# itshawi/data-accelerator

Hardware: AMD Instinct MI355X
Metric: events/sec (node) + p99 latency, SimulatedData IoT Flow (higher is better)
Workload: dtype fp64/int64 columns (no reduced precision)

## Files before the change

### dxa/io/kafka_device.py

```python
from __future__ import annotations

import ctypes
from dataclasses import dataclass
from typing import List, Optional, Sequence, Tuple

import numpy as np
import torch

_PLAN_ERRS = {-2: "message format is not v2", -3: "CRC mismatch", -5: "codec decoded on the host only",
              -7: "malformed compressed payload (LZ4 / snappy / zstd)", -8: "dependent-block LZ4 frame", -9: "offset deltas with gaps"}


TORCH_DT = {np.dtype(np.int32): torch.int32, np.dtype(np.int64): torch.int64, np.dtype(np.uint8): torch.uint8}


class Unsupported(Exception):
    """The fetch needs the host decoder."""


_BOUND = False


def _lib():
    global _BOUND
# ... 213 lines not shown
    keep[cut] = max_records - before
    keep[cut + 1:] = 0
    q = FetchPlan(**{**p.__dict__, "b_keep": keep.astype(np.int32)})
    q.b_rec0 = _rec0(q)
    q.next_offset = int(p.b_base[cut] + p.b_skip[cut] + keep[cut])
    return q


class DeviceRecordDecoder:

    def __init__(self, device, chunks: int = 4, copy_stream=None, decode_stream=None, track: bool = True,
                 verify_crc: bool = False):
        self.device = torch.device(device)
        self.verify_crc = verify_crc
        self.crc_stream = torch.cuda.Stream(self.device) if verify_crc else None
        self.chunks = max(1, chunks)
        cus = torch.cuda.get_device_properties(self.device).multi_processor_count
        self.min_blocks_per_chunk = cus * 64
        self.copy_stream = copy_stream or torch.cuda.Stream(self.device)
        self.decode_stream = decode_stream or torch.cuda.Stream(self.device)
        self.track = track
        self.checks: List["DecodeStatus"] = []

    def decode(self, staging: torch.Tensor, plan: FetchPlan):
        from ..engine.processor import RawBatch
        from ..ops import native as N
        dev = self.device
        n = plan.nrec
        if plan.packed is None:
            if not hasattr(self, "_packs"):
                self._packs = PlanBufferPool()
            pb = self._packs.get()
            plan.buffer = pb
            arrs, layout, used = pb.carve(plan.nbat, plan.nblk)
            for name, _dt, _k in _ARRAYS:
                arrs[name][...] = getattr(plan, name)
            packed = pb.buf[:used]
        else:
            packed, layout = plan.packed, plan.layout
        with torch.cuda.stream(self.copy_stream):
            dtab = packed.to(dev, non_blocking=True)
            ddata = torch.empty(plan.nbytes + 32, dtype=torch.uint8, device=dev)
            tab_ev = torch.cuda.Event()
            tab_ev.record(self.copy_stream)
        if getattr(plan, "buffer", None) is not None:
            plan.buffer.release(tab_ev)
        views = {name: dtab[off:off + cnt * np.dtype(dt).itemsize].view(TORCH_DT[np.dtype(dt)])
                 for (name, off, cnt), (_, dt, _k) in zip(layout, _ARRAYS)}
        tabs = [views[k] for k in ("k_comp_off", "k_comp_len", "k_stored", "k_out_off", "k_cap", "b_count",
                                   "b_skip", "b_keep", "b_first", "b_nblk", "b_rec0")]
        crc_tabs = [views[k] for k in ("b_crc_off", "b_crc_len", "b_crc")]
        co, cl, sd, oo, cap, bc, bs, bk, bf, bn, br = tabs
        with torch.cuda.stream(self.decode_stream):
            out = torch.empty(plan.out_bytes + 64, dtype=torch.uint8, device=dev)
            produced = torch.empty(max(1, plan.nblk), dtype=torch.int64, device=dev)
            bstat = torch.empty(max(1, plan.nblk), dtype=torch.int32, device=dev)
            offs = torch.empty(n + 1, dtype=torch.int64, device=dev)
            ends = torch.empty(max(1, n), dtype=torch.int64, device=dev)
            rstat = torch.empty(max(1, plan.nbat), dtype=torch.int32, device=dev)
        self.decode_stream.wait_event(tab_ev)
        st = self.decode_stream.cuda_stream
        nb = plan.nblk
        chunks = max(1, min(self.chunks, nb // max(1, self.min_blocks_per_chunk)))
        kinds = set(np.unique(plan.k_stored[:nb]).tolist()) if nb else set()
        has_gzip, has_snappy, has_zstd = 2 in kinds, 3 in kinds, 4 in kinds
        bounds = np.linspace(0, nb, chunks + 1).astype(np.int64)
        ev_last = tab_ev
        copied = 0
        for k in range(chunks):
            b0, b1 = int(bounds[k]), int(bounds[k + 1])
            if b1 <= b0:
                continue
            lo = copied
            hi = plan.nbytes if b1 == nb else int(plan.k_comp_off[b1])
            copied = hi
            N.call("dxa_memcpy_h2d_async", ddata.data_ptr() + lo, staging.data_ptr() + lo, hi - lo,
                   self.copy_stream.cuda_stream)
            ev = torch.cuda.Event()
            ev.record(self.copy_stream)
            ev_last = ev
            self.decode_stream.wait_event(ev)
            N.call("dxa_lz4_decode_into", N.ptr(ddata), N.ptr(co[b0:b1]), N.ptr(cl[b0:b1]), N.ptr(sd[b0:b1]),
                   N.ptr(oo[b0:b1]), N.ptr(cap[b0:b1]), b1 - b0, N.ptr(out), N.ptr(produced[b0:b1]),
                   N.ptr(bstat[b0:b1]), st)
            for present, entry in ((has_gzip, "dxa_inflate_into"), (has_snappy, "dxa_snappy_decode_into"),
                                   (has_zstd, "dxa_zstd_decode_into")):
                if present:
                    N.call(entry, N.ptr(ddata), N.ptr(co[b0:b1]), N.ptr(cl[b0:b1]), N.ptr(sd[b0:b1]),
                           N.ptr(oo[b0:b1]), N.ptr(cap[b0:b1]), b1 - b0, N.ptr(out), N.ptr(produced[b0:b1]),
                           N.ptr(bstat[b0:b1]), st)
        with torch.cuda.stream(self.decode_stream):
            offs[n:].fill_(plan.out_bytes)
        N.call("dxa_kafka_records", N.ptr(out), plan.nbat, N.ptr(bc), N.ptr(bs), N.ptr(bk), N.ptr(bf), N.ptr(bn),
               N.ptr(br), N.ptr(oo), N.ptr(cap), N.ptr(produced), N.ptr(bstat), N.ptr(offs), N.ptr(ends),
               N.ptr(rstat), st)
        done = torch.cuda.Event()
        done.record(self.decode_stream)
        if self.verify_crc:
            cs = self.crc_stream
            cs.wait_event(ev_last)
            with torch.cuda.stream(cs):
                cstat = torch.empty(max(1, plan.nbat), dtype=torch.int32, device=dev)
            N.call("dxa_kafka_crc", N.ptr(ddata), plan.nbat, *[N.ptr(t) for t in crc_tabs], N.ptr(cstat),
                   cs.cuda_stream)
            cs.wait_event(done)
            with torch.cuda.stream(cs):
                bad = (rstat[:plan.nbat] != 0).sum() + (cstat[:plan.nbat] != 0).sum()
                status = DecodeStatus(bad, cs)
            for t in (ddata, dtab, rstat):
                t.record_stream(cs)
        else:
            with torch.cuda.stream(self.decode_stream):
                status = DecodeStatus((rstat[:plan.nbat] != 0).sum(), self.decode_stream)
        for t in (ddata, produced, bstat, dtab):
            t.record_stream(self.decode_stream)
        if self.track:
            self.checks.append(status)
        self._inflight = [(e, b) for e, b in getattr(self, "_inflight", []) if not e.query()] + \
            [(status.event if self.verify_crc else done, (staging, packed))]
        return RawBatch(out, offs, n, ends=ends[:n], source_bytes=plan.nbytes, status=status), done

    def check(self):
        pending, self.checks = self.checks, []
        bad = sum(s.failed() for s in pending)
        if bad:
            raise DecodeError(f"{bad} Kafka record batch(es) failed to decode on the device")


class DecodeError(ValueError):
    pass


class DecodeStatus:

    __slots__ = ("host", "event")

    def __init__(self, bad: torch.Tensor, stream):
        self.host = torch.empty(1, dtype=torch.int64, pin_memory=True)
        self.host.copy_(bad.reshape(1), non_blocking=True)
        self.event = torch.cuda.Event()
        self.event.record(stream)

    def failed(self) -> int:
        self.event.synchronize()
        return int(self.host[0])

    def raise_if_failed(self, what: str = "batch"):
        bad = self.failed()
        if bad:
            raise DecodeError(f"{what}: {bad} Kafka record batch(es) failed to decode on the device")


_CRC_POLY = 0x82F63B78


def _multmodp(a: int, b: int) -> int:
    p = 0
    m = 1 << 31
    while m:
        if a & m:
            p ^= b
        b = (b >> 1) ^ _CRC_POLY if b & 1 else b >> 1
        m >>= 1
    return p


def _x2n_table():
# ... 116 lines not shown
```

### dxa/ops/csrc/lz4.hip

```cpp
#include "dxa_common.h"

namespace {

struct InWin {
  const uint8_t* base;
  uintptr_t wb;
  uint4 w;
  __device__ __forceinline__ uint32_t at(int64_t q) {
    const uintptr_t a = reinterpret_cast<uintptr_t>(base + q);
    const uintptr_t b = a & ~(uintptr_t)15;
    if (b != wb) {
      wb = b;
      w = *reinterpret_cast<const uint4*>(b);
    }
    return dxa::window_byte(w, (uint32_t)(a - b));
  }
};

struct OutBuf {
  uint8_t* p;
  int64_t len;
  int head;
  int nacc;
  uint64_t a0, a1;
// ... 27 lines not shown
      const int k = (int)(q - acc0);
      return (uint32_t)(((k < 8) ? (a0 >> (8 * k)) : (a1 >> (8 * (k - 8)))) & 0xff);
    }
    const uintptr_t a = reinterpret_cast<uintptr_t>(p + q);
    const uintptr_t b = a & ~(uintptr_t)15;
    if (b != wb) {
      wb = b;
      asm volatile("" ::: "memory");
      w = *reinterpret_cast<const uint4*>(b);
    }
    return dxa::window_byte(w, (uint32_t)(a - b));
  }
  __device__ __forceinline__ void finish() {
    uint8_t* q = p + len - nacc;
    for (int k = 0; k < nacc; ++k) q[k] = (uint8_t)((k < 8 ? a0 >> (8 * k) : a1 >> (8 * (k - 8))) & 0xff);
  }
};

enum : int32_t { LZ_OK = 0, LZ_TRUNC = 1, LZ_OFFSET = 2, LZ_OVERFLOW = 3, LZ_SIZE = 4 };

template <bool WRITE>
__device__ int32_t run_block(const uint8_t* src, int64_t n, uint8_t* dst, int64_t cap, int64_t& produced) {
  InWin in{src, 0, make_uint4(0, 0, 0, 0)};
  OutBuf out;
  if (WRITE) out.init(dst);
  int64_t ip = 0, op = 0;
  while (ip < n) {
    const uint32_t token = in.at(ip++);
    int64_t lit = token >> 4;
    if (lit == 15) {
      uint32_t b;
      do { if (ip >= n) return LZ_TRUNC; b = in.at(ip++); lit += b; } while (b == 255);
    }
    if (lit > n - ip) return LZ_TRUNC;
    if (lit > cap - op) return LZ_OVERFLOW;
    if (WRITE) for (int64_t k = 0; k < lit; ++k) out.put(in.at(ip + k));
    ip += lit;
    op += lit;
    if (ip >= n) break;
    if (n - ip < 2) return LZ_TRUNC;
    const int64_t off = (int64_t)in.at(ip) | ((int64_t)in.at(ip + 1) << 8);
    ip += 2;
    if (off == 0 || off > op) return LZ_OFFSET;
    int64_t ml = token & 15;
    if (ml == 15) {
      uint32_t b;
      do { if (ip >= n) return LZ_TRUNC; b = in.at(ip++); ml += b; } while (b == 255);
    }
    ml += 4;
    if (ml > cap - op) return LZ_OVERFLOW;
    if (WRITE) {
      const int64_t s = op - off;
      if (off == 1) {
        const uint32_t c = out.get(s);
        for (int64_t k = 0; k < ml; ++k) out.put(c);
      } else {
        for (int64_t k = 0; k < ml; ++k) out.put(out.get(s + k));
      }
    }
    op += ml;
  }
  if (WRITE) out.finish();
  produced = op;
  return LZ_OK;
}

__global__ __launch_bounds__(256) void lz4_sizes_kernel(const uint8_t* __restrict__ src,
                                                        const int64_t* __restrict__ comp_off,
                                                        const int32_t* __restrict__ comp_len,
                                                        const uint8_t* __restrict__ stored, int64_t nb,
                                                        int64_t max_block, int64_t* __restrict__ out_len,
                                                        int32_t* __restrict__ status) {
  const int64_t b = (int64_t)blockIdx.x * blockDim.x + threadIdx.x;
  if (b >= nb) return;
  if (stored[b]) { out_len[b] = comp_len[b]; status[b] = LZ_OK; return; }
  int64_t produced = 0;
  const int32_t rc = run_block<false>(src + comp_off[b], comp_len[b], nullptr, max_block, produced);
  out_len[b] = rc == LZ_OK ? produced : 0;
  status[b] = rc;
}

constexpr int kWaitVm0 = 0xF70;

template <int G>
__global__ __launch_bounds__(256) void lz4_decode_group_kernel(const uint8_t* __restrict__ src,
                                                               const int64_t* __restrict__ comp_off,
                                                               const int32_t* __restrict__ comp_len,
                                                               const uint8_t* __restrict__ stored,
                                                               const int64_t* __restrict__ out_off,
                                                               const int64_t* __restrict__ out_len, int64_t nb,
                                                               uint8_t* __restrict__ dst,
                                                               int32_t* __restrict__ status,
                                                               int64_t* __restrict__ produced) {
  static_assert(G == 8 || G == 16, "group width");
  constexpr int NW = 16 / G, LPL = 16 / G, BPL = 32 / G, LOG_G = G == 8 ? 3 : 4;
  constexpr int WB = 64, PIPE = 32;
  const int64_t b = ((int64_t)blockIdx.x * 256 + threadIdx.x) / G;
  const int gl = (int)(threadIdx.x & (G - 1));
  const int gbase = (int)((threadIdx.x & 63) & ~(G - 1));
  if (b >= nb) return;
  const uint8_t kd = stored[b];
  if (kd > 1) return;
  const int32_t n = comp_len[b];
  const int64_t cap64 = out_len[b];
  const uint8_t* in = src + comp_off[b];
  uint8_t* out = dst + out_off[b];
  auto put = [&](bool on, int32_t pos, uint32_t v) {
    if (on) out[pos] = (uint8_t)v;
  };
  auto fetch = [&](bool on, int32_t pos) -> uint32_t { return on ? (uint32_t)out[pos] : 0u; };
  if (kd) {
    if (produced ? (n > cap64) : (n != cap64)) {
      if (gl == 0) status[b] = LZ_SIZE;
      return;
    }
    for (int32_t k = gl; k < n; k += G) out[k] = in[k];
    if (gl == 0) {
      status[b] = LZ_OK;
      if (produced) produced[b] = n;
    }
    return;
  }
  if (cap64 > INT32_MAX || cap64 < 0 || n < 0) {
    if (gl == 0) status[b] = LZ_OVERFLOW;
    return;
  }
  const int32_t cap = (int32_t)cap64;
  const int32_t shift = (int32_t)(reinterpret_cast<uintptr_t>(in) & 3);
  const uint8_t* a0 = in - shift;
  const int32_t lim = shift + n + 16;
  uint32_t X[NW];
  auto ld = [&](int32_t w0) {
#pragma unroll
    for (int k = 0; k < NW; ++k) {
      const int32_t q = w0 + 4 * (gl + G * k);
      X[k] = (q + 4 <= lim) ? *reinterpret_cast<const uint32_t*>(a0 + q) : 0u;
    }
    __builtin_amdgcn_s_waitcnt(kWaitVm0);
  };
  auto wbyte = [&](int32_t r) -> uint32_t {
    const int d = (r >> 2) & (G * NW - 1);
    const int addr = (gbase + (d & (G - 1))) << 2;
    uint32_t v = (uint32_t)__builtin_amdgcn_ds_bpermute(addr, (int)X[0]);
    if constexpr (NW == 2) {
      const uint32_t v1 = (uint32_t)__builtin_amdgcn_ds_bpermute(addr, (int)X[1]);
      v = (d >> LOG_G) ? v1 : v;
    }
    return (v >> ((r & 3) * 8)) & 0xffu;
  };
  int32_t xb = 0;
  ld(0);
  auto get = [&](int32_t p) -> uint32_t {
    if (p - xb >= WB) {
      xb = p & ~3;
      ld(xb);
    }
    return wbyte(p - xb);
  };
  const int32_t iend = shift + n;
  int32_t ip = shift, op = 0, rc = LZ_OK, done = 0;
  int32_t pdst = 0, pml = 0;
  uint32_t pv[BPL];
#pragma unroll
  for (int k = 0; k < BPL; ++k) pv[k] = 0;
  auto flush = [&]() {
#pragma unroll
    for (int k = 0; k < BPL; ++k) put(gl + G * k < pml, pdst + G * k + gl, pv[k]);
  };
  while (ip < iend) {
    if (ip - xb > WB - 16) {
      xb = ip & ~3;
      ld(xb);
    }
    const int32_t r = ip - xb;
    const uint32_t token = wbyte(r);
    int32_t lit = (int32_t)(token >> 4);
    const int32_t mlc = (int32_t)(token & 15);
    const bool has_ext = mlc == 15 && lit < 15 && r + lit + 4 <= WB;
    const uint32_t mext = has_ext ? wbyte(r + lit + 3) : 0u;
    const int32_t fml = mlc + 4 + (int32_t)mext;
    const int32_t fhdr = lit + 3 + (mlc == 15 ? 1 : 0);
    if (lit < 15 && (mlc < 15 || mext < 255) && r + fhdr <= WB && iend - ip >= fhdr && cap - op >= lit + fml) {
#pragma unroll
      for (int k = 0; k < LPL; ++k) {
        const uint32_t lv = wbyte(r + 1 + G * k + gl);
        put(gl + G * k < lit, op + G * k + gl, lv);
      }
      const int32_t off = (int32_t)(wbyte(r + 1 + lit) | (wbyte(r + 2 + lit) << 8));
      ip += fhdr;
      op += lit;
      if (off == 0 || off > op) { rc = LZ_OFFSET; break; }
      const int32_t ml = fml;
      const int32_t s0 = op - off;
      const int32_t src_end = s0 + (off < ml ? off : ml);
      if (pml > 0 && (src_end > pdst || ml > PIPE)) {
        flush();
        pml = 0;
      }
      if (src_end > done) {
        __builtin_amdgcn_s_waitcnt(kWaitVm0);
        asm volatile("" ::: "memory");
        done = pml > 0 ? pdst : op;
      }
      if (ml > PIPE) {
        if (off >= ml) {
          for (int32_t c = 0; c < ml; c += G)
            if (c + gl < ml) out[op + c + gl] = out[s0 + c + gl];
        } else {
          for (int32_t c = 0; c < ml; c += G) {
            const uint32_t i = (uint32_t)(c + gl);
            if ((int32_t)i < ml) out[op + i] = out[s0 + (int32_t)(i % (uint32_t)off)];
          }
        }
        op += ml;
        continue;
      }
      uint32_t v[BPL];
      if (off >= ml) {
#pragma unroll
        for (int k = 0; k < BPL; ++k) v[k] = fetch(gl + G * k < ml, s0 + G * k + gl);
      } else {
        const uint32_t o = (uint32_t)off;
#pragma unroll
        for (int k = 0; k < BPL; ++k) v[k] = fetch(gl + G * k < ml, s0 + (int32_t)((uint32_t)(gl + G * k) % o));
      }
      if (pml > 0) flush();
      pdst = op;
      pml = ml;
#pragma unroll
      for (int k = 0; k < BPL; ++k) pv[k] = v[k];
      op += ml;
      continue;
    }
    if (pml > 0) {
      flush();
      pml = 0;
    }
    ++ip;
    if (lit == 15) {
      uint32_t e;
      do {
        if (ip >= iend) { rc = LZ_TRUNC; break; }
        e = get(ip);
        ++ip;
        lit += (int32_t)e;
      } while (e == 255);
      if (rc != LZ_OK) break;
    }
    if (lit > iend - ip) { rc = LZ_TRUNC; break; }
    if (lit > cap - op) { rc = LZ_OVERFLOW; break; }
    for (int32_t c = 0; c < lit; c += G)
      if (c + gl < lit) out[op + c + gl] = a0[ip + c + gl];
    ip += lit;
    op += lit;
    if (ip >= iend) break;
    if (iend - ip < 2) { rc = LZ_TRUNC; break; }
    const int32_t off = (int32_t)(get(ip) | (get(ip + 1) << 8));
    ip += 2;
    if (off == 0 || off > op) { rc = LZ_OFFSET; break; }
    int32_t ml = mlc;
    if (ml == 15) {
      uint32_t e;
      do {
        if (ip >= iend) { rc = LZ_TRUNC; break; }
        e = get(ip);
        ++ip;
        ml += (int32_t)e;
      } while (e == 255);
      if (rc != LZ_OK) break;
    }
    ml += 4;
    if (ml > cap - op) { rc = LZ_OVERFLOW; break; }
    const int32_t s0 = op - off;
    if (s0 + (off < ml ? off : ml) > done) {
      __builtin_amdgcn_s_waitcnt(kWaitVm0);
      asm volatile("" ::: "memory");
      done = op;
    }
    if (off >= ml) {
      for (int32_t c = 0; c < ml; c += G)
        if (c + gl < ml) out[op + c + gl] = out[s0 + c + gl];
    } else {
      for (int32_t c = 0; c < ml; c += G) {
        const uint32_t i = (uint32_t)(c + gl);
        if ((int32_t)i < ml) out[op + i] = out[s0 + (int32_t)(i % (uint32_t)off)];
      }
    }
    op += ml;
  }
  if (pml > 0) flush();
  if (rc == LZ_OK && !produced && op != cap) rc = LZ_SIZE;
  if (gl == 0) {
    status[b] = rc;
    if (produced) produced[b] = op;
  }
}

}

DXA_API int dxa_lz4_block_sizes(const void* src, const void* comp_off, const void* comp_len, const void* stored,
                                int64_t nb, int64_t max_block, void* out_len, void* status, void* st) {
  if (nb <= 0) return 0;
  hipLaunchKernelGGL(lz4_sizes_kernel, dim3((unsigned)((nb + 255) / 256)), dim3(256), 0, (hipStream_t)st,
                     (const uint8_t*)src, (const int64_t*)comp_off, (const int32_t*)comp_len, (const uint8_t*)stored,
                     nb, max_block, (int64_t*)out_len, (int32_t*)status);
  return (int)hipGetLastError();
}

template <int G>
static int launch_group(int64_t nb, hipStream_t s, const uint8_t* src, const int64_t* co, const int32_t* cl,
                        const uint8_t* sd, const int64_t* oo, const int64_t* ol, uint8_t* dst, int32_t* status,
                        int64_t* produced) {
  const dim3 grid((unsigned)((nb * G + 255) / 256));
  hipLaunchKernelGGL((lz4_decode_group_kernel<G>), grid, dim3(256), 0, s, src, co, cl, sd, oo, ol, nb, dst, status,
                     produced);
  return (int)hipGetLastError();
}

DXA_API int dxa_lz4_decode(const void* src, const void* comp_off, const void* comp_len, const void* stored,
                           const void* out_off, const void* out_len, int64_t nb, int64_t max_out, void* dst,
                           void* status, void* st) {
  if (nb <= 0) return 0;
  const hipStream_t s = (hipStream_t)st;
  return launch_group<16>(nb, s, (const uint8_t*)src, (const int64_t*)comp_off, (const int32_t*)comp_len,
                          (const uint8_t*)stored, (const int64_t*)out_off, (const int64_t*)out_len, (uint8_t*)dst,
                          (int32_t*)status, (int64_t*)nullptr);
}

DXA_API int dxa_lz4_decode_into(const void* src, const void* comp_off, const void* comp_len, const void* stored,
                                const void* out_off, const void* cap, int64_t nb, void* dst, void* produced,
                                void* status, void* st) {
  if (nb <= 0) return 0;
  const hipStream_t s = (hipStream_t)st;
  const uint8_t* s8 = (const uint8_t*)src;
  const int64_t* co = (const int64_t*)comp_off;
  const int32_t* cl = (const int32_t*)comp_len;
  const uint8_t* sd = (const uint8_t*)stored;
  const int64_t* oo = (const int64_t*)out_off;
  const int64_t* cp = (const int64_t*)cap;
  return launch_group<16>(nb, s, s8, co, cl, sd, oo, cp, (uint8_t*)dst, (int32_t*)status, (int64_t*)produced);
}

DXA_API int dxa_memcpy_h2d_async(void* dst, const void* src, int64_t n, void* st) {
  if (n <= 0) return 0;
  return (int)hipMemcpyAsync(dst, src, (size_t)n, hipMemcpyHostToDevice, (hipStream_t)st);
}
```

### dxa/ops/lz4.py

```python
from __future__ import annotations

import ctypes
import os
from dataclasses import dataclass
from typing import Optional

import numpy as np
import torch

from . import native as N

DEFAULT_BLOCK = 16 * 1024
_HOST = None


class Lz4Error(RuntimeError):
    pass


def _host():
    global _HOST
    if _HOST is None:
        from .serialize import lib
        L = lib()
# ... 102 lines not shown
            return None
        return off, ln


def frame_table(data) -> FrameTable:
    a = _as_np(data)
    L = _host()
    cs, mb, fe = ctypes.c_int64(0), ctypes.c_int32(0), ctypes.c_int64(0)
    nb = L.dxa_lz4_frame_blocks(a.ctypes.data, a.size, None, None, None, 0, ctypes.byref(cs), ctypes.byref(mb),
                                ctypes.byref(fe))
    if nb == -2:
        raise Lz4Error("dependent-block or dictionary LZ4 frames are decoded on the host only")
    if nb < 0:
        raise Lz4Error("malformed LZ4 frame")
    off = np.zeros(nb, dtype=np.int64)
    ln = np.zeros(nb, dtype=np.int32)
    st = np.zeros(nb, dtype=np.uint8)
    L.dxa_lz4_frame_blocks(a.ctypes.data, a.size, off.ctypes.data, ln.ctypes.data, st.ctypes.data, nb,
                           ctypes.byref(cs), ctypes.byref(mb), ctypes.byref(fe))
    return FrameTable(off, ln, st, cs.value, mb.value, fe.value)


@dataclass
class DeviceFrame:
    data: torch.Tensor
    comp_off: torch.Tensor
    comp_len: torch.Tensor
    stored: torch.Tensor
    out_off: Optional[torch.Tensor]
    out_len: Optional[torch.Tensor]
    content_size: int
    max_block: int
    max_out: int = -1

    @staticmethod
    def from_frame(frame: np.ndarray, block_size: Optional[int] = DEFAULT_BLOCK, pin: bool = False) -> "DeviceFrame":
        t = frame_table(frame)
        padded = np.zeros(frame.size + 32, dtype=np.uint8)
        padded[:frame.size] = frame
        oo = t.out_offsets(block_size)

        def T(x):
            x = torch.from_numpy(np.ascontiguousarray(x))
            return x.pin_memory() if pin else x
        return DeviceFrame(T(padded), T(t.comp_off), T(t.comp_len), T(t.stored),
                           T(oo[0]) if oo else None, T(oo[1]) if oo else None, t.content_size, t.max_block,
                           int(oo[1].max()) if oo and oo[1].size else -1)

    def to(self, device, non_blocking: bool = True) -> "DeviceFrame":
        f = lambda x: None if x is None else x.to(device, non_blocking=non_blocking)
        return DeviceFrame(f(self.data), f(self.comp_off), f(self.comp_len), f(self.stored), f(self.out_off),
                           f(self.out_len), self.content_size, self.max_block, self.max_out)

    def tensors(self):
        return [x for x in (self.data, self.comp_off, self.comp_len, self.stored, self.out_off, self.out_len)
                if x is not None]


def decompress_device(fr: DeviceFrame, check: bool = False) -> torch.Tensor:
    dev = fr.data.device
    if dev.type != "cuda":
        raw = decompress_frame(fr.data.numpy()[:-32])
        out = torch.zeros(len(raw) + 16, dtype=torch.uint8)
        out[:len(raw)] = torch.frombuffer(bytearray(raw), dtype=torch.uint8)
        return out
    nb = int(fr.comp_off.shape[0])
    st = N.stream_handle(dev)
    status = torch.empty(max(nb, 1), dtype=torch.int32, device=dev)
    if fr.out_off is None:
        ln = torch.empty(max(nb, 1), dtype=torch.int64, device=dev)
        N.call("dxa_lz4_block_sizes", N.ptr(fr.data), N.ptr(fr.comp_off), N.ptr(fr.comp_len), N.ptr(fr.stored), nb,
               fr.max_block, N.ptr(ln), N.ptr(status), st)
        ln = ln[:nb]
        off = torch.cumsum(ln, 0) - ln
        total = int(ln.sum().item()) if nb else 0
        max_out = int(ln.max().item()) if nb else 0
        if nb and bool((status[:nb] != 0).any()):
            raise Lz4Error("malformed LZ4 block")
    else:
        off, ln, total, max_out = fr.out_off, fr.out_len, fr.content_size, fr.max_out
    out = torch.empty(total + 16, dtype=torch.uint8, device=dev)
    out[total:].zero_()
    N.call("dxa_lz4_decode", N.ptr(fr.data), N.ptr(fr.comp_off), N.ptr(fr.comp_len), N.ptr(fr.stored), N.ptr(off),
           N.ptr(ln), nb, max_out, N.ptr(out), N.ptr(status), st)
    if check and nb and bool((status[:nb] != 0).any()):
        raise Lz4Error(f"LZ4 block decode failed: status {status[:nb].unique().tolist()}")
    return out


class ChunkedIngest:

    def __init__(self, device, chunks: int = 8, copy_stream=None, decode_stream=None):
        self.device = device
        self.chunks = max(1, chunks)
        self.copy_stream = copy_stream or torch.cuda.Stream(device)
        self.decode_stream = decode_stream or torch.cuda.Stream(device)

    def stage(self, fr: "DeviceFrame"):
        dev = self.device
        if fr.out_off is None:
            raise Lz4Error("chunked ingest needs frames with known block sizes")
        nb = int(fr.comp_off.shape[0])
        total = fr.content_size
        with torch.cuda.stream(self.decode_stream):
            out = torch.empty(total + 16, dtype=torch.uint8, device=dev)
            status = torch.empty(max(nb, 1), dtype=torch.int32, device=dev)
        with torch.cuda.stream(self.copy_stream):
            ddata = torch.empty(fr.data.shape[0], dtype=torch.uint8, device=dev)
        with torch.cuda.stream(self.copy_stream):
            tabs = [x.to(dev, non_blocking=True) for x in (fr.comp_off, fr.comp_len, fr.stored, fr.out_off,
                                                           fr.out_len)]
            tab_ev = torch.cuda.Event()
            tab_ev.record(self.copy_stream)
        comp_off_h = fr.comp_off.numpy() if fr.comp_off.device.type == "cpu" else fr.comp_off.cpu().numpy()
        bounds = np.linspace(0, nb, self.chunks + 1).astype(np.int64)
        nbytes = int(fr.data.shape[0])
        st = self.decode_stream.cuda_stream
        self.decode_stream.wait_event(tab_ev)
        with torch.cuda.stream(self.decode_stream):
            out[total:].zero_()
        for k in range(self.chunks):
            b0, b1 = int(bounds[k]), int(bounds[k + 1])
            if b1 <= b0:
                continue
            lo = 0 if k == 0 else int(comp_off_h[b0])
            hi = nbytes if b1 == nb else int(comp_off_h[b1])
            if fr.data.device.type == "cpu":
                if not fr.data.is_pinned():
                    raise Lz4Error("chunked ingest needs a pinned host frame")
                N.call("dxa_memcpy_h2d_async", ddata.data_ptr() + lo, fr.data.data_ptr() + lo, hi - lo,
                       self.copy_stream.cuda_stream)
            else:
                with torch.cuda.stream(self.copy_stream):
                    ddata[lo:hi].copy_(fr.data[lo:hi], non_blocking=True)
            ev = torch.cuda.Event()
            ev.record(self.copy_stream)
            self.decode_stream.wait_event(ev)
            co, cl, sd, oo, ol = tabs
            N.call("dxa_lz4_decode", N.ptr(ddata), N.ptr(co[b0:b1]), N.ptr(cl[b0:b1]), N.ptr(sd[b0:b1]),
                   N.ptr(oo[b0:b1]), N.ptr(ol[b0:b1]), b1 - b0, fr.max_out, N.ptr(out), N.ptr(status[b0:b1]), st)
        done = torch.cuda.Event()
        done.record(self.decode_stream)
        for t in (ddata, *tabs):
            t.record_stream(self.decode_stream)
        self._inflight = [(e, f) for e, f in getattr(self, "_inflight", []) if not e.query()] + [(done, fr)]
        return out, done
```

### dxa/ops/native.py

```python
from __future__ import annotations

import ctypes
import os
import threading
from pathlib import Path

import torch

_LIB = None
_LOCK = threading.Lock()
_HERE = Path(__file__).resolve().parent
LIB_PATH = Path(os.environ.get("DXA_NATIVE_LIB") or (_HERE / "_native" / "libdxa_kernels.so"))

c_i64 = ctypes.c_int64
c_i32 = ctypes.c_int32
c_p = ctypes.c_void_p

_SIGS = {
    "dxa_byte_map": [c_p, c_p, c_i64, c_p, c_p],
    "dxa_lz4_block_sizes": [c_p, c_p, c_p, c_p, c_i64, c_i64, c_p, c_p, c_p],
    "dxa_lz4_decode": [c_p, c_p, c_p, c_p, c_p, c_p, c_i64, c_i64, c_p, c_p, c_p],
    "dxa_memcpy_h2d_async": [c_p, c_p, c_i64, c_p],
    "dxa_copy_sdma": [c_p, c_p, c_i64],
    "dxa_lz4_decode_into": [c_p, c_p, c_p, c_p, c_p, c_p, c_i64, c_p, c_p, c_p, c_p],
    "dxa_inflate_into": [c_p, c_p, c_p, c_p, c_p, c_p, c_i64, c_p, c_p, c_p, c_p],
    "dxa_snappy_decode_into": [c_p, c_p, c_p, c_p, c_p, c_p, c_i64, c_p, c_p, c_p, c_p],
    "dxa_zstd_decode_into": [c_p, c_p, c_p, c_p, c_p, c_p, c_i64, c_p, c_p, c_p, c_p],
    "dxa_zstd_decode_prof": [c_p, c_p, c_p, c_p, c_p, c_p, c_i64, c_p, c_p, c_p, c_p, c_p],
    "dxa_kafka_records": [c_p, c_i64] + [c_p] * 14,
    "dxa_kafka_crc": [c_p, c_i64, c_p, c_p, c_p, c_p, c_p],
    "dxa_csv_tokenize": [c_p, c_p, c_i64, c_i32, c_i32, c_i32, c_i32, c_p, c_p, c_p, c_p, c_p],
    "dxa_spark_hash_fixed": [c_p, c_i32, c_p, c_i64, c_p, c_p],
    "dxa_spark_hash_str": [c_p, c_p, c_p, c_p, c_i64, c_p, c_p],
    "dxa_serialize_rows": [c_i32, c_p, c_i32, c_i32, c_i32, c_p, c_p, c_p, c_p, c_p],
    "dxa_java_double_dev": [c_p, c_i64, c_p, c_p, c_p],
    "dxa_java_double_hostcheck": [c_p, c_i64, c_p, c_p],
    "dxa_json_parse": [c_p, c_p, c_i64, c_p, c_p, c_i32, c_p, c_p, c_p, c_i32, c_p, c_p, c_p, c_p,
                       c_p, c_p, c_p, c_p, c_p, c_i32, c_p, c_p, c_p, c_p, c_i32, c_i32, c_i32, c_p, c_i32,
                       c_p],
    "dxa_count_newlines": [c_p, c_i64, c_i64, c_p, c_p, c_p],
    "dxa_write_newlines_bits": [c_p, c_i64, c_i64, c_p, c_p, c_i64, c_i64, c_p],
    "dxa_null_counts": [c_p, c_i64, c_i32, c_p, c_p],
    "dxa_hash_i64": [c_p, c_p, c_i64, c_p, ctypes.c_int, c_p],
    "dxa_hash_f64": [c_p, c_p, c_i64, c_p, ctypes.c_int, c_p],
    "dxa_hash_str": [c_p, c_p, c_p, c_p, c_i64, c_p, ctypes.c_int, c_p],
    "dxa_table_insert": [c_p, c_i64, c_p, c_i64, c_p, c_p],
    "dxa_group_ids": [c_p, c_i64, c_p, c_i64, c_p, c_p, c_p, c_p, c_p],
    "dxa_verify_i64": [c_p, c_p, c_p, c_p, c_i64, c_p, c_p],
    "dxa_verify_f64": [c_p, c_p, c_p, c_p, c_i64, c_p, c_p],
    "dxa_verify_str": [c_p, c_p, c_p, c_p, c_p, c_p, c_i64, c_p, c_p],
    "dxa_aggregate": [c_p, c_p, c_p, c_i64, c_i32, c_i32, c_i32, c_p, c_p],
    "dxa_aggregate_multi": [c_p, c_i64, c_i32, c_i32, c_p, c_i32, c_p, c_p, c_p],
    "dxa_aggregate_finish": [c_p, c_i32, c_i32, c_i32, c_p, c_p, c_p, c_p],
    "dxa_partial_finish_size": [],
    "dxa_partial_finish": [c_p, c_p],
    "dxa_group_renumber": [c_p, c_i64, c_p, c_i32, c_p, c_p, c_p],
    "dxa_group_build": [c_p, c_i64, c_p, c_i64, c_p, c_p, c_p, c_p, c_p],
    "dxa_group_build_init": [c_p, c_i64, c_p, c_i64, c_p, c_p, c_p, c_p, c_p],
    "dxa_slot_count": [c_p, c_i64, c_p, c_p],
    "dxa_slot_scatter": [c_p, c_i64, c_p, c_p, c_p, c_p],
    "dxa_probe_count": [c_p, c_p, c_i64, c_p, c_i64, c_p, c_p, c_p, ctypes.c_int, c_p],
    "dxa_probe_write": [c_p, c_i64, c_p, c_p, c_p, c_p, c_p, c_p, ctypes.c_int, c_p],
    "dxa_str_cmp_lit": [c_p, c_p, c_p, c_i64, c_p, c_i32, c_i32, c_p, c_p],
    "dxa_str_eq_col": [c_p, c_p, c_p, c_p, c_p, c_p, c_i64, c_p, c_p],
    "dxa_str_cmp_col": [c_p, c_p, c_p, c_p, c_p, c_p, c_i64, c_i32, c_p, c_p],
    "dxa_str_gather": [c_p, c_p, c_p, c_i64, c_p, c_p, c_p],
    "dxa_str_gather_parts": [c_p, c_i32, c_p],
    "dxa_str_split_count": [c_p, c_p, c_p, c_i64, c_p, c_i32, c_p, c_p],
    "dxa_ts_format": [c_p, c_i64, c_p, c_i32, c_p, c_i32, c_p, c_p],
    "dxa_str_like": [c_p, c_p, c_p, c_i64, c_p, c_i32, c_p, c_p],
    "dxa_str_rlike": [c_p, c_p, c_p, c_i64, c_p, c_i32, c_i32, c_i32, c_p, c_p],
    "dxa_str_regex": [c_p, c_p, c_p, c_i64, c_p, c_i32, c_p, c_i32, c_i32, c_i32, c_p, c_i32, c_p, c_p, c_p, c_p, c_p,
                      c_p, c_p],
    "dxa_gzip_chunks": [c_p, c_i64, c_i32, c_p, c_p, c_i32, c_p, c_p],
    "dxa_gzip_pack": [c_p, c_i32, c_p, c_p, c_i64, c_p, c_p],
    "dxa_str_digest": [c_p, c_p, c_p, c_i64, c_i32, c_p, c_p],
    "dxa_str_crc32": [c_p, c_p, c_p, c_i64, c_p, c_p],
    "dxa_str_encode": [c_p, c_p, c_p, c_i64, c_i32, c_p, c_p, c_p],
    "dxa_f64_str_len": [c_p, c_p, c_i64, c_p, c_p],
    "dxa_f64_str_write": [c_p, c_p, c_i64, c_p, c_p, c_p],
    "dxa_str_to_num": [c_p, c_p, c_p, c_p, c_i64, c_i32, c_p, c_p, c_p],
    "dxa_concat_ws_len": [c_p, c_i32, c_i64, c_i32, c_p, c_p],
    "dxa_concat_ws_write": [c_p, c_i32, c_i64, c_p, c_i32, c_p, c_p, c_p],
    "dxa_str_substr": [c_p, c_p, c_p, c_i64, c_p, c_i64, c_p, c_i64, c_p, c_p, c_p],
    "dxa_str_trim": [c_p, c_p, c_p, c_i64, c_i32, c_p, c_p, c_p],
    "dxa_str_numchars": [c_p, c_p, c_p, c_i64, c_p, c_p],
    "dxa_str_locate": [c_p, c_p, c_p, c_i64, c_p, c_i32, c_i64, c_p, c_p],
    "dxa_str_replace_len": [c_p, c_p, c_p, c_i64, c_p, c_i32, c_i32, c_p, c_p],
    "dxa_str_replace_write": [c_p, c_p, c_p, c_i64, c_p, c_i32, c_p, c_i32, c_p, c_p, c_p],
    "dxa_str_split_write": [c_p, c_p, c_p, c_i64, c_p, c_i32, c_i32, c_p, c_p, c_p],
    "dxa_str_part_size": [],
    "dxa_concat_len": [c_p, c_i32, c_i64, c_p, c_p, c_p],
    "dxa_concat_write": [c_p, c_i32, c_i64, c_p, c_p, c_p, c_p],
    "dxa_concat_part_size": [],
    "dxa_i64_to_str_len": [c_p, c_i64, c_p, c_p],
    "dxa_i64_to_str_write": [c_p, c_i64, c_p, c_p, c_p],
    "dxa_i64_to_str_slots": [c_p, c_i64, c_p, c_p, c_p, c_p],
    "dxa_case_map": [c_p, c_p, c_p, c_i64, c_p, c_p, ctypes.c_int, c_p],
    "dxa_str_to_ts": [c_p, c_p, c_p, c_p, c_i64, c_p, c_p, c_p],
    "dxa_datagen_op_size": [],
    "dxa_datagen_lengths": [c_p, c_i32, c_p, c_i32, c_p, c_i32, ctypes.c_uint64, c_i64, c_i64, c_i64, c_i64, c_p,
                            c_p],
    "dxa_datagen_write": [c_p, c_i32, c_p, c_i32, c_p, c_i32, ctypes.c_uint64, c_i64, c_i64, c_i64, c_i64, c_p,
                          c_p, c_p],
}

_OPTIONAL_SIGS = {}
# ... 106 lines not shown
```

Measured before the change: 252.3 million.

## Rework LZ4 group decoder with LDS input window and 32-bit addressing

The LZ4 group decode kernel now stages its 64-byte input window in shared memory instead of sharing it across lanes with ds_bpermute. It adds a templated 32-bit offset addressing mode on global address-space pointers, chosen at launch when the buffers fit in 4 GiB. The fast-path sequence loop is restructured: the token, literal, offset and extension bytes are read speculatively up front, the pending match is always flushed, bad offsets are handled without branching, and the slow path moves into a helper lambda. The aim is to cut address arithmetic, cross-lane permute cost and branch divergence, at the price of LDS use per block, which can lower occupancy, and extra launch parameters threaded through the Python callers.

```diff
diff --git a/dxa/io/kafka_device.py b/dxa/io/kafka_device.py
--- a/dxa/io/kafka_device.py
+++ b/dxa/io/kafka_device.py
@@ -319,7 +319,7 @@
             self.decode_stream.wait_event(ev)
             N.call("dxa_lz4_decode_into", N.ptr(ddata), N.ptr(co[b0:b1]), N.ptr(cl[b0:b1]), N.ptr(sd[b0:b1]),
                    N.ptr(oo[b0:b1]), N.ptr(cap[b0:b1]), b1 - b0, N.ptr(out), N.ptr(produced[b0:b1]),
-                   N.ptr(bstat[b0:b1]), st)
+                   N.ptr(bstat[b0:b1]), st, ddata.numel(), out.numel(), 0)
             for present, entry in ((has_gzip, "dxa_inflate_into"), (has_snappy, "dxa_snappy_decode_into"),
                                    (has_zstd, "dxa_zstd_decode_into")):
                 if present:
diff --git a/dxa/ops/csrc/lz4.hip b/dxa/ops/csrc/lz4.hip
--- a/dxa/ops/csrc/lz4.hip
+++ b/dxa/ops/csrc/lz4.hip
@@ -133,7 +133,9 @@
 
 constexpr int kWaitVm0 = 0xF70;
 
-template <int G>
+#define G1 __attribute__((address_space(1)))
+
+template <int G, bool A32>
 __global__ __launch_bounds__(256) void lz4_decode_group_kernel(const uint8_t* __restrict__ src,
                                                                const int64_t* __restrict__ comp_off,
                                                                const int32_t* __restrict__ comp_len,
@@ -144,28 +146,52 @@
                                                                int32_t* __restrict__ status,
                                                                int64_t* __restrict__ produced) {
   static_assert(G == 8 || G == 16, "group width");
-  constexpr int NW = 16 / G, LPL = 16 / G, BPL = 32 / G, LOG_G = G == 8 ? 3 : 4;
-  constexpr int WB = 64, PIPE = 32;
+  constexpr int NW = 16 / G, LPL = 16 / G, BPL = 32 / G;
+  constexpr int WB = 64, PIPE = 32, FH = 18;
+  __shared__ __attribute__((aligned(16))) uint8_t win[(256 / G) * WB + 4];
   const int64_t b = ((int64_t)blockIdx.x * 256 + threadIdx.x) / G;
   const int gl = (int)(threadIdx.x & (G - 1));
-  const int gbase = (int)((threadIdx.x & 63) & ~(G - 1));
+  const uint32_t wb = (threadIdx.x / G) * WB;
   if (b >= nb) return;
   const uint8_t kd = stored[b];
   if (kd > 1) return;
   const int32_t n = comp_len[b];
   const int64_t cap64 = out_len[b];
-  const uint8_t* in = src + comp_off[b];
-  uint8_t* out = dst + out_off[b];
+  const int64_t co = comp_off[b], oo = out_off[b];
+  const int32_t shift = (int32_t)(A32 ? (uint64_t)co & 3 : reinterpret_cast<uintptr_t>(src + co) & 3);
+  const G1 uint8_t* src_g = (const G1 uint8_t*)src;
+  G1 uint8_t* dst_g = (G1 uint8_t*)dst;
+  const uint32_t ib = (uint32_t)co - (uint32_t)shift, ob = (uint32_t)oo;
+  const G1 uint8_t* a0 = src_g + (co - shift);
+  G1 uint8_t* out = dst_g + oo;
+  auto in8 = [&](int32_t q) -> uint32_t {
+    if constexpr (A32) return src_g[ib + (uint32_t)q];
+    else return a0[q];
+  };
+  auto in32 = [&](int32_t q) -> uint32_t {
+    if constexpr (A32) return *reinterpret_cast<const G1 uint32_t*>(src_g + (ib + (uint32_t)q));
+    else return *reinterpret_cast<const G1 uint32_t*>(a0 + q);
+  };
+  auto out8 = [&](int32_t pos) -> uint32_t {
+    if constexpr (A32) return dst_g[ob + (uint32_t)pos];
+    else return out[pos];
+  };
+  auto st8 = [&](int32_t pos, uint32_t v) {
+    if constexpr (A32) dst_g[ob + (uint32_t)pos] = (uint8_t)v;
+    else out[pos] = (uint8_t)v;
+  };
   auto put = [&](bool on, int32_t pos, uint32_t v) {
-    if (on) out[pos] = (uint8_t)v;
-  };
-  auto fetch = [&](bool on, int32_t pos) -> uint32_t { return on ? (uint32_t)out[pos] : 0u; };
+    if (on) st8(pos, v);
+  };
+  auto fetch = [&](bool on, int32_t pos, uint32_t& v) {
+    if (on) v = out8(pos);
+  };
   if (kd) {
     if (produced ? (n > cap64) : (n != cap64)) {
       if (gl == 0) status[b] = LZ_SIZE;
       return;
     }
-    for (int32_t k = gl; k < n; k += G) out[k] = in[k];
+    for (int32_t k = gl; k < n; k += G) st8(k, in8(shift + k));
     if (gl == 0) {
       status[b] = LZ_OK;
       if (produced) produced[b] = n;
@@ -177,28 +203,16 @@
     return;
   }
   const int32_t cap = (int32_t)cap64;
-  const int32_t shift = (int32_t)(reinterpret_cast<uintptr_t>(in) & 3);
-  const uint8_t* a0 = in - shift;
   const int32_t lim = shift + n + 16;
-  uint32_t X[NW];
   auto ld = [&](int32_t w0) {
 #pragma unroll
     for (int k = 0; k < NW; ++k) {
       const int32_t q = w0 + 4 * (gl + G * k);
-      X[k] = (q + 4 <= lim) ? *reinterpret_cast<const uint32_t*>(a0 + q) : 0u;
-    }
-    __builtin_amdgcn_s_waitcnt(kWaitVm0);
-  };
-  auto wbyte = [&](int32_t r) -> uint32_t {
-    const int d = (r >> 2) & (G * NW - 1);
-    const int addr = (gbase + (d & (G - 1))) << 2;
-    uint32_t v = (uint32_t)__builtin_amdgcn_ds_bpermute(addr, (int)X[0]);
-    if constexpr (NW == 2) {
-      const uint32_t v1 = (uint32_t)__builtin_amdgcn_ds_bpermute(addr, (int)X[1]);
-      v = (d >> LOG_G) ? v1 : v;
-    }
-    return (v >> ((r & 3) * 8)) & 0xffu;
-  };
+      const uint32_t x = (q + 4 <= lim) ? in32(q) : 0u;
+      *reinterpret_cast<uint32_t*>(win + wb + 4 * (gl + G * k)) = x;
+    }
+  };
+  auto wbyte = [&](int32_t r) -> uint32_t { return win[wb + (uint32_t)r]; };
   int32_t xb = 0;
   ld(0);
   auto get = [&](int32_t p) -> uint32_t {
@@ -218,126 +232,121 @@
 #pragma unroll
     for (int k = 0; k < BPL; ++k) put(gl + G * k < pml, pdst + G * k + gl, pv[k]);
   };
-  while (ip < iend) {
-    if (ip - xb > WB - 16) {
-      xb = ip & ~3;
-      ld(xb);
-    }
-    const int32_t r = ip - xb;
-    const uint32_t token = wbyte(r);
-    int32_t lit = (int32_t)(token >> 4);
-    const int32_t mlc = (int32_t)(token & 15);
-    const bool has_ext = mlc == 15 && lit < 15 && r + lit + 4 <= WB;
-    const uint32_t mext = has_ext ? wbyte(r + lit + 3) : 0u;
-    const int32_t fml = mlc + 4 + (int32_t)mext;
-    const int32_t fhdr = lit + 3 + (mlc == 15 ? 1 : 0);
-    if (lit < 15 && (mlc < 15 || mext < 255) && r + fhdr <= WB && iend - ip >= fhdr && cap - op >= lit + fml) {
-#pragma unroll
-      for (int k = 0; k < LPL; ++k) {
-        const uint32_t lv = wbyte(r + 1 + G * k + gl);
-        put(gl + G * k < lit, op + G * k + gl, lv);
-      }
-      const int32_t off = (int32_t)(wbyte(r + 1 + lit) | (wbyte(r + 2 + lit) << 8));
-      ip += fhdr;
-      op += lit;
-      if (off == 0 || off > op) { rc = LZ_OFFSET; break; }
-      const int32_t ml = fml;
-      const int32_t s0 = op - off;
-      const int32_t src_end = s0 + (off < ml ? off : ml);
-      if (pml > 0 && (src_end > pdst || ml > PIPE)) {
-        flush();
-        pml = 0;
-      }
-      if (src_end > done) {
-        __builtin_amdgcn_s_waitcnt(kWaitVm0);
-        asm volatile("" ::: "memory");
-        done = pml > 0 ? pdst : op;
-      }
-      if (ml > PIPE) {
-        if (off >= ml) {
-          for (int32_t c = 0; c < ml; c += G)
-            if (c + gl < ml) out[op + c + gl] = out[s0 + c + gl];
-        } else {
-          for (int32_t c = 0; c < ml; c += G) {
-            const uint32_t i = (uint32_t)(c + gl);
-            if ((int32_t)i < ml) out[op + i] = out[s0 + (int32_t)(i % (uint32_t)off)];
-          }
-        }
-        op += ml;
-        continue;
-      }
-      uint32_t v[BPL];
-      if (off >= ml) {
-#pragma unroll
-        for (int k = 0; k < BPL; ++k) v[k] = fetch(gl + G * k < ml, s0 + G * k + gl);
-      } else {
-        const uint32_t o = (uint32_t)off;
-#pragma unroll
-        for (int k = 0; k < BPL; ++k) v[k] = fetch(gl + G * k < ml, s0 + (int32_t)((uint32_t)(gl + G * k) % o));
-      }
-      if (pml > 0) flush();
-      pdst = op;
-      pml = ml;
-#pragma unroll
-      for (int k = 0; k < BPL; ++k) pv[k] = v[k];
-      op += ml;
-      continue;
-    }
-    if (pml > 0) {
-      flush();
-      pml = 0;
-    }
+  auto copy_match = [&](int32_t s0, int32_t off, int32_t ml) {
+    if (off >= ml) {
+      for (int32_t c = 0; c < ml; c += G)
+        if (c + gl < ml) st8(op + c + gl, out8(s0 + c + gl));
+    } else {
+      for (int32_t c = 0; c < ml; c += G) {
+        const uint32_t i = (uint32_t)(c + gl);
+        if ((int32_t)i < ml) st8(op + (int32_t)i, out8(s0 + (int32_t)(i % (uint32_t)off)));
+      }
+    }
+  };
+  auto general = [&](int32_t lit, int32_t mlc) -> int32_t {
     ++ip;
     if (lit == 15) {
       uint32_t e;
       do {
-        if (ip >= iend) { rc = LZ_TRUNC; break; }
+        if (ip >= iend) return LZ_TRUNC;
         e = get(ip);
         ++ip;
         lit += (int32_t)e;
       } while (e == 255);
-      if (rc != LZ_OK) break;
-    }
-    if (lit > iend - ip) { rc = LZ_TRUNC; break; }
-    if (lit > cap - op) { rc = LZ_OVERFLOW; break; }
+    }
+    if (lit > iend - ip) return LZ_TRUNC;
+    if (lit > cap - op) return LZ_OVERFLOW;
     for (int32_t c = 0; c < lit; c += G)
-      if (c + gl < lit) out[op + c + gl] = a0[ip + c + gl];
+      if (c + gl < lit) st8(op + c + gl, in8(ip + c + gl));
     ip += lit;
     op += lit;
-    if (ip >= iend) break;
-    if (iend - ip < 2) { rc = LZ_TRUNC; break; }
+    if (ip >= iend) return LZ_OK;
+    if (iend - ip < 2) return LZ_TRUNC;
     const int32_t off = (int32_t)(get(ip) | (get(ip + 1) << 8));
     ip += 2;
-    if (off == 0 || off > op) { rc = LZ_OFFSET; break; }
+    if (off == 0 || off > op) return LZ_OFFSET;
     int32_t ml = mlc;
     if (ml == 15) {
       uint32_t e;
       do {
-        if (ip >= iend) { rc = LZ_TRUNC; break; }
+        if (ip >= iend) return LZ_TRUNC;
         e = get(ip);
         ++ip;
         ml += (int32_t)e;
       } while (e == 255);
-      if (rc != LZ_OK) break;
     }
     ml += 4;
-    if (ml > cap - op) { rc = LZ_OVERFLOW; break; }
+    if (ml > cap - op) return LZ_OVERFLOW;
     const int32_t s0 = op - off;
     if (s0 + (off < ml ? off : ml) > done) {
       __builtin_amdgcn_s_waitcnt(kWaitVm0);
       asm volatile("" ::: "memory");
       done = op;
     }
-    if (off >= ml) {
-      for (int32_t c = 0; c < ml; c += G)
-        if (c + gl < ml) out[op + c + gl] = out[s0 + c + gl];
+    copy_match(s0, off, ml);
+    op += ml;
+    return LZ_OK;
+  };
+  while (ip < iend) {
+    if (ip - xb > WB - FH) {
+      xb = ip & ~3;
+      ld(xb);
+    }
+    const int32_t r = ip - xb;
+    uint32_t token = wbyte(r);
+    uint32_t lv[LPL];
+#pragma unroll
+    for (int k = 0; k < LPL; ++k) {
+      lv[k] = wbyte(r + 1 + G * k + gl);
+      asm volatile("" : "+v"(lv[k]));
+    }
+    const int32_t lit = (int32_t)(token >> 4);
+    const int32_t mlc = (int32_t)(token & 15);
+    uint32_t off_lo = wbyte(r + 1 + lit), off_hi = wbyte(r + 2 + lit), ext = wbyte(r + 3 + lit);
+    asm volatile("" : "+v"(off_lo), "+v"(off_hi), "+v"(ext));
+    const uint32_t mext = mlc == 15 ? ext : 0u;
+    const int32_t fml = mlc + 4 + (int32_t)mext;
+    const int32_t fhdr = lit + 3 + (mlc == 15 ? 1 : 0);
+    flush();
+    pml = 0;
+    if (lit < 15 && mext < 255 && iend - ip >= fhdr && cap - op >= lit + fml) {
+#pragma unroll
+      for (int k = 0; k < LPL; ++k) put(gl + G * k < lit, op + G * k + gl, lv[k]);
+      const int32_t off = (int32_t)(off_lo | (off_hi << 8));
+      op += lit;
+      const bool bad = off == 0 || off > op;
+      const int32_t ml = bad ? 0 : fml;
+      rc = bad ? (int32_t)LZ_OFFSET : rc;
+      ip = bad ? iend : ip + fhdr;
+      const int32_t s0 = op - off;
+      const int32_t src_end = s0 + (off < ml ? off : ml);
+      if (src_end > done) {
+        __builtin_amdgcn_s_waitcnt(kWaitVm0);
+        asm volatile("" ::: "memory");
+        done = op;
+      }
+      if (ml > PIPE) {
+        copy_match(s0, off, ml);
+      } else {
+        if (off >= ml) {
+#pragma unroll
+          for (int k = 0; k < BPL; ++k) fetch(gl + G * k < ml, s0 + G * k + gl, pv[k]);
+        } else {
+          const uint32_t o = (uint32_t)off;
+#pragma unroll
+          for (int k = 0; k < BPL; ++k) fetch(gl + G * k < ml, s0 + (int32_t)((uint32_t)(gl + G * k) % o), pv[k]);
+        }
+        pdst = op;
+        pml = ml;
+      }
+      op += ml;
     } else {
-      for (int32_t c = 0; c < ml; c += G) {
-        const uint32_t i = (uint32_t)(c + gl);
-        if ((int32_t)i < ml) out[op + i] = out[s0 + (int32_t)(i % (uint32_t)off)];
-      }
-    }
-    op += ml;
+      const int32_t e = general(lit, mlc);
+      if (e != LZ_OK) {
+        rc = e;
+        ip = iend;
+      }
+    }
   }
   if (pml > 0) flush();
   if (rc == LZ_OK && !produced && op != cap) rc = LZ_SIZE;
@@ -358,29 +367,39 @@
   return (int)hipGetLastError();
 }
 
+constexpr int64_t kMax32 = ((int64_t)1 << 32) - 64;
+
 template <int G>
 static int launch_group(int64_t nb, hipStream_t s, const uint8_t* src, const int64_t* co, const int32_t* cl,
                         const uint8_t* sd, const int64_t* oo, const int64_t* ol, uint8_t* dst, int32_t* status,
-                        int64_t* produced) {
+                        int64_t* produced, int64_t src_bytes, int64_t dst_bytes, int32_t addressing) {
+  const bool fits = src_bytes > 0 && dst_bytes > 0 && src_bytes <= kMax32 && dst_bytes <= kMax32 &&
+                    (reinterpret_cast<uintptr_t>(src) & 3) == 0;
+  if ((addressing != 0 && addressing != 32 && addressing != 64) || (addressing == 32 && !fits))
+    return (int)hipErrorInvalidValue;
   const dim3 grid((unsigned)((nb * G + 255) / 256));
-  hipLaunchKernelGGL((lz4_decode_group_kernel<G>), grid, dim3(256), 0, s, src, co, cl, sd, oo, ol, nb, dst, status,
-                     produced);
+  if (addressing == 64 ? false : fits)
+    hipLaunchKernelGGL((lz4_decode_group_kernel<G, true>), grid, dim3(256), 0, s, src, co, cl, sd, oo, ol, nb, dst,
+                       status, produced);
+  else
+    hipLaunchKernelGGL((lz4_decode_group_kernel<G, false>), grid, dim3(256), 0, s, src, co, cl, sd, oo, ol, nb, dst,
+                       status, produced);
   return (int)hipGetLastError();
 }
 
 DXA_API int dxa_lz4_decode(const void* src, const void* comp_off, const void* comp_len, const void* stored,
                            const void* out_off, const void* out_len, int64_t nb, int64_t max_out, void* dst,
-                           void* status, void* st) {
+                           void* status, void* st, int64_t src_bytes, int64_t dst_bytes, int32_t addressing) {
   if (nb <= 0) return 0;
   const hipStream_t s = (hipStream_t)st;
   return launch_group<16>(nb, s, (const uint8_t*)src, (const int64_t*)comp_off, (const int32_t*)comp_len,
                           (const uint8_t*)stored, (const int64_t*)out_off, (const int64_t*)out_len, (uint8_t*)dst,
-                          (int32_t*)status, (int64_t*)nullptr);
+                          (int32_t*)status, (int64_t*)nullptr, src_bytes, dst_bytes, addressing);
 }
 
 DXA_API int dxa_lz4_decode_into(const void* src, const void* comp_off, const void* comp_len, const void* stored,
                                 const void* out_off, const void* cap, int64_t nb, void* dst, void* produced,
-                                void* status, void* st) {
+                                void* status, void* st, int64_t src_bytes, int64_t dst_bytes, int32_t addressing) {
   if (nb <= 0) return 0;
   const hipStream_t s = (hipStream_t)st;
   const uint8_t* s8 = (const uint8_t*)src;
@@ -389,7 +408,8 @@
   const uint8_t* sd = (const uint8_t*)stored;
   const int64_t* oo = (const int64_t*)out_off;
   const int64_t* cp = (const int64_t*)cap;
-  return launch_group<16>(nb, s, s8, co, cl, sd, oo, cp, (uint8_t*)dst, (int32_t*)status, (int64_t*)produced);
+  return launch_group<16>(nb, s, s8, co, cl, sd, oo, cp, (uint8_t*)dst, (int32_t*)status, (int64_t*)produced,
+                          src_bytes, dst_bytes, addressing);
 }
 
 DXA_API int dxa_memcpy_h2d_async(void* dst, const void* src, int64_t n, void* st) {
diff --git a/dxa/ops/lz4.py b/dxa/ops/lz4.py
--- a/dxa/ops/lz4.py
+++ b/dxa/ops/lz4.py
@@ -208,7 +208,7 @@
     out = torch.empty(total + 16, dtype=torch.uint8, device=dev)
     out[total:].zero_()
     N.call("dxa_lz4_decode", N.ptr(fr.data), N.ptr(fr.comp_off), N.ptr(fr.comp_len), N.ptr(fr.stored), N.ptr(off),
-           N.ptr(ln), nb, max_out, N.ptr(out), N.ptr(status), st)
+           N.ptr(ln), nb, max_out, N.ptr(out), N.ptr(status), st, fr.data.numel(), out.numel(), 0)
     if check and nb and bool((status[:nb] != 0).any()):
         raise Lz4Error(f"LZ4 block decode failed: status {status[:nb].unique().tolist()}")
     return out
@@ -264,7 +264,8 @@
             self.decode_stream.wait_event(ev)
             co, cl, sd, oo, ol = tabs
             N.call("dxa_lz4_decode", N.ptr(ddata), N.ptr(co[b0:b1]), N.ptr(cl[b0:b1]), N.ptr(sd[b0:b1]),
-                   N.ptr(oo[b0:b1]), N.ptr(ol[b0:b1]), b1 - b0, fr.max_out, N.ptr(out), N.ptr(status[b0:b1]), st)
+                   N.ptr(oo[b0:b1]), N.ptr(ol[b0:b1]), b1 - b0, fr.max_out, N.ptr(out), N.ptr(status[b0:b1]), st,
+                   nbytes, out.numel(), 0)
         done = torch.cuda.Event()
         done.record(self.decode_stream)
         for t in (ddata, *tabs):
diff --git a/dxa/ops/native.py b/dxa/ops/native.py
--- a/dxa/ops/native.py
+++ b/dxa/ops/native.py
@@ -19,10 +19,10 @@
 _SIGS = {
     "dxa_byte_map": [c_p, c_p, c_i64, c_p, c_p],
     "dxa_lz4_block_sizes": [c_p, c_p, c_p, c_p, c_i64, c_i64, c_p, c_p, c_p],
-    "dxa_lz4_decode": [c_p, c_p, c_p, c_p, c_p, c_p, c_i64, c_i64, c_p, c_p, c_p],
+    "dxa_lz4_decode": [c_p, c_p, c_p, c_p, c_p, c_p, c_i64, c_i64, c_p, c_p, c_p, c_i64, c_i64, c_i32],
     "dxa_memcpy_h2d_async": [c_p, c_p, c_i64, c_p],
     "dxa_copy_sdma": [c_p, c_p, c_i64],
-    "dxa_lz4_decode_into": [c_p, c_p, c_p, c_p, c_p, c_p, c_i64, c_p, c_p, c_p, c_p],
+    "dxa_lz4_decode_into": [c_p, c_p, c_p, c_p, c_p, c_p, c_i64, c_p, c_p, c_p, c_p, c_i64, c_i64, c_i32],
     "dxa_inflate_into": [c_p, c_p, c_p, c_p, c_p, c_p, c_i64, c_p, c_p, c_p, c_p],
     "dxa_snappy_decode_into": [c_p, c_p, c_p, c_p, c_p, c_p, c_i64, c_p, c_p, c_p, c_p],
     "dxa_zstd_decode_into": [c_p, c_p, c_p, c_p, c_p, c_p, c_i64, c_p, c_p, c_p, c_p],
```

Result: no change. 251.2 million (-0.4%).
